# ayankele/dune-transformercvn

Hardware: AMD Instinct MI355X
Metric: events/sec (fwd+bwd) at batch=32, 8 prongs/event; fraction of MFMA roofline (higher is better)
Workload: dtype bf16; 1 GPU; TransformerCVN DenseNet [3,6,12,6,3] g32, fwd+loss+bwd, batch 32/GPU, 8 prongs/event, 3x400x280 maps, 6-layer encoder, dropout 0.1; global_batch=32, parallelism=dp1, precision=bf16

## Files before the change

### dune-transformercvn_amd/csrc/densenet.hip

```cpp
#include <string>
#include <vector>
#include <cstring>

#include "tcvn_rows.h"
#include <cstdlib>
#include "densenet_plan.h"

using namespace tcvn;

namespace {
constexpr float kEps = 1e-5f, kMom = 0.1f;
}

int DenseNetPlan::add_slot(const std::string& name, long numel, int kind) {
    slots.push_back({name, numel, kind});
    return (int)slots.size() - 1;
}
BnSlots DenseNetPlan::add_bn(const std::string& p, int c) {
    BnSlots s;
    s.w = add_slot(p + ".weight", c, TCVN_SLOT_PARAM);
    s.b = add_slot(p + ".bias", c, TCVN_SLOT_PARAM);
    s.rm = add_slot(p + ".running_mean", c, TCVN_SLOT_BUFFER);
    s.rv = add_slot(p + ".running_var", c, TCVN_SLOT_BUFFER);
    s.nbt = add_slot(p + ".num_batches_tracked", 1, TCVN_SLOT_COUNTER);
// ... 23 lines not shown
            const std::string p = f + ".dense" + std::to_string(b + 1) + ".layers." + std::to_string(l);
            ls.n1 = add_bn(p + ".bottleneck_block.norm1", cin);
            ls.a1 = add_slot(p + ".bottleneck_block.relu1.weight", cin, TCVN_SLOT_PARAM);
            ls.w1 = add_slot(p + ".bottleneck_block.conv1.weight", (long)mid * cin, TCVN_SLOT_PARAM);
            ls.b1 = add_slot(p + ".bottleneck_block.conv1.bias", mid, TCVN_SLOT_PARAM);
            ls.n2 = add_bn(p + ".output_block.norm2", mid);
            ls.a2 = add_slot(p + ".output_block.relu2.weight", mid, TCVN_SLOT_PARAM);
            ls.w2 = add_slot(p + ".output_block.conv2.weight", (long)g * mid * 9, TCVN_SLOT_PARAM);
            ls.b2 = add_slot(p + ".output_block.conv2.bias", g, TCVN_SLOT_PARAM);
            ls.cin = cin;
            bg.layers.push_back(ls);
        }
        ch = bg.Ctot;
        if (b != cfg.n_blocks - 1) {
            const std::string p = f + ".transition" + std::to_string(b + 1);
            bg.has_trans = true;
            bg.tn = add_bn(p + ".norm", ch);
            bg.ta = add_slot(p + ".relu.weight", ch, TCVN_SLOT_PARAM);
            bg.tw = add_slot(p + ".conv.weight", (long)(ch / 2) * ch, TCVN_SLOT_PARAM);
            bg.tb = add_slot(p + ".conv.bias", ch / 2, TCVN_SLOT_PARAM);
            ch = ch / 2; h = h / 2; w = w / 2;
        }
        blocks.push_back(bg);
    }
    Cf = ch;
    nf = add_bn(f + ".final_norm", ch);
    s_af = add_slot(f + ".final_relu.weight", ch, TCVN_SLOT_PARAM);
    s_wl = add_slot("output_block.linear.weight", (long)cfg.out_dim * ch, TCVN_SLOT_PARAM);
    nl = add_bn("output_block.norm", cfg.out_dim);
    s_al = add_slot("output_block.relu.weight", cfg.out_dim, TCVN_SLOT_PARAM);
    data.assign(slots.size(), nullptr);
    grad.assign(slots.size(), nullptr);
    for (const auto& bg : blocks) path.emplace_back(bg.L);
}

DenseNetPlan::~DenseNetPlan() {
    if (d_desc) (void)hipFree(d_desc);
    if (d_undesc) (void)hipFree(d_undesc);
    if (side_st) {
        (void)hipStreamSynchronize(side_st);
        (void)hipStreamDestroy(side_st);
        (void)hipEventDestroy(ev_fork_a); (void)hipEventDestroy(ev_fork_b); (void)hipEventDestroy(ev_done[0]);
        (void)hipEventDestroy(ev_done[1]); (void)hipEventDestroy(ev_drain);
    }
}
int DenseNetPlan::ensure_side() {
    if (side_st) return 0;
    TCVN_CHECK(hipStreamCreateWithFlags(&side_st, hipStreamNonBlocking));
    hipEvent_t* evs[5] = {&ev_fork_a, &ev_fork_b, &ev_done[0], &ev_done[1], &ev_drain};
    for (hipEvent_t* e : evs) TCVN_CHECK(hipEventCreateWithFlags(e, hipEventDisableTiming));
    return 0;
}

namespace {
struct Bump {
    long off = 0;
    long take(long bytes) { long o = off; off += round_up(bytes, 256); return o; }
};
}

void DenseNetPlan::layout(int n, bool bwd, Layout& L) const {
    Bump b;
    const int mid = cfg.bn_size * cfg.growth;
    L.img = b.take((long)n * cfg.H * cfg.W * cfg.in_ch * esz);
    L.c0 = b.take((long)n * Hc * Wc * cfg.init_ch * esz);
    L.D.clear(); L.Y.clear(); L.bstatD.clear(); L.bstatY.clear(); L.YA.clear(); L.XA.clear(); L.XP.clear(); L.KM.clear();
// ... 446 lines not shown
        if (!p.fuse_ya) {
            ActArgs act{Y, mid, M, mid, a.sc, a.sh, a.sl, s.ws + L.YA[bi][l], mid};
            if ((rc = act_bf16(act, s.st))) return rc;
        }
        a.Aact = s.ws + L.YA[bi][l];
    }
    a.part = s.train ? s.part : nullptr;
    a.drop_p = s.train ? cfg.dropout : 0.f; a.seed = s.seed; a.stream_id = (uint32_t)(bi * 64 + l + 1);
    a.nblk = conv_fwd_nblk(a);
    if (p.lf2) {
        if (!a.act_fused) { fprintf(stderr, "tcvn: link-free norm2 without the in-LDS activation\n"); return -17; }
        a.lf = lf_link(s, ls.n2, isumY, 2L * mid, 0, mid, bstatY, M);
    }
    if (p.out_isum) { a.isum_out = isumD + 2 * ls.cin; a.isum_stride = 2L * bg.ld; }
    if (s.train && !L.KM[bi].empty()) a.keep_out = reinterpret_cast<uint32_t*>(s.ws + L.KM[bi][l]);
    if ((rc = conv_fwd(a, s.st))) return rc;
    fr = FreshStats{ls.cin, g, a.nblk, g, p.out_isum};
    return 0;
}

int DenseNetPlan::fwd_transition(const Step& s, int bi, FreshStats& fr) {
    const Layout& L = s.L;
    const BlockGeom& bg = blocks[bi];
    char* D = s.ws + L.D[bi];
    int rc;
    if ((rc = link_fresh(s, bg.has_trans ? bg.tn : nf, bi, fr))) return rc;
    if (!bg.has_trans) {
        const Tab t = tab(s.ws, L, nf);
        HeadPoolArgs a{cfg.mode, D, bg.ld, s.n, bg.H * bg.W, Cf, t.sc, t.sh, data[s_af], reinterpret_cast<float*>(s.ws + L.F)};
        return head_pool_fwd(a, s.st);
    }
    const BlockGeom& nb = blocks[bi + 1];
    fr = FreshStats{0, nb.C0, 0, bg.Ctot / 2, false};
    if (L.XP[bi] >= 0) {
        const Tab t = tab(s.ws, L, bg.tn);
        ActPoolArgs ap{D, bg.ld, s.n, bg.H, bg.W, bg.Ctot, t.sc, t.sh, data[bg.ta], s.ws + L.XP[bi], bg.ldp};
        if ((rc = cfg.mode == MODE_BF16 ? act_pool_bf16(ap, s.st) : act_pool_f32(ap, s.st))) return rc;
    }
    if (L.XP[bi] >= 0 && cfg.mode == MODE_BF16) {
        const WkEntry& ef = wk_find(bg.tw, 0, 1);
        GemmNtArgs ga{};
        ga.epi = EPI_FWD; ga.A = s.ws + L.XP[bi]; ga.lda = bg.ldp; ga.K = bg.ldp; ga.M = (long)s.n * nb.H * nb.W; ga.N = bg.Ctot / 2;
        ga.Wfrag = s.ws + L.wk + ef.off; ga.Kp = ef.Kp; ga.zeros = s.ws + L.zeros; ga.bias = data[bg.tb];
        ga.Out = s.ws + L.D[bi + 1]; ga.ldo = nb.ld; ga.n_off = 0; ga.part = s.train ? s.part : nullptr; ga.nblk = gemm_nt_nblk(ga);
        if ((rc = gemm_nt_bf16(ga, "k_gemm_nt_bf16<fwdtrans>", s.st))) return rc;
        fr.nblk = ga.nblk;
        return 0;
    }
    ConvFwdArgs a = trans_args(s, bi);
    a.part = s.train ? s.part : nullptr; a.nblk = conv_fwd_nblk(a);
    if ((rc = conv_fwd(a, s.st))) return rc;
    fr.nblk = a.nblk;
    return 0;
}

int DenseNetPlan::fwd_output(const Step& s, float* out, long out_ld) const {
    float* F = reinterpret_cast<float*>(s.ws + s.L.F);
    float* Z = reinterpret_cast<float*>(s.ws + s.L.Z);
    int rc;
    if ((rc = linear_fwd(F, Cf, data[s_wl], nullptr, Z, cfg.out_dim, s.n, cfg.out_dim, Cf, s.st))) return rc;
    float* hs = reinterpret_cast<float*>(s.ws + s.L.head_stat);
    RowsBnArgs r{};
    r.X = Z; r.ldx = cfg.out_dim; r.R = s.n; r.C = cfg.out_dim; r.gamma = data[nl.w]; r.beta = data[nl.b]; r.slope = data[s_al];
    r.running_mean = data[nl.rm]; r.running_var = data[nl.rv]; r.Y = out; r.ldy = out_ld;
    r.save_mean = hs; r.save_rstd = hs + cfg.out_dim; r.train = s.train; r.eps = kEps; r.momentum = kMom;
    r.drop_p = s.train ? cfg.dropout : 0.f; r.seed = s.seed; r.stream_id = 0x4000u;
// ... 2 lines not shown

int DenseNetPlan::tap(int n, const char* name, long* off, int* tn, int* th, int* tw, int* tc, int* tld, int* tes) const {
    Layout L;
    layout(n, false, L);
    std::string s(name);
    *tn = n; *tes = esz;
    if ((s == "img" || s == "conv0") && stem_path.sparse && n == last_n) return -1;
    if (s == "img") { *off = L.img; *th = cfg.H; *tw = cfg.W; *tc = cfg.in_ch; *tld = cfg.in_ch; return 0; }
    if (s == "conv0") { *off = L.c0; *th = Hc; *tw = Wc; *tc = cfg.init_ch; *tld = cfg.init_ch; return 0; }
    if (s == "condense") { *off = L.F; *th = 1; *tw = 1; *tc = Cf; *tld = Cf; *tes = 4; return 0; }
    if (s == "raw:wk") { *tn = *th = *tw = 1; *off = L.wk; *tc = *tld = (int)(wk_bytes() / esz); return 0; }
    if (s == "raw:tabs") { *tn = *th = *tw = 1; *off = L.tabs; *tc = *tld = (int)tab_floats(); *tes = 4; return 0; }
    if (s.rfind("raw:ystat", 0) == 0) {
        int b = 0, l = 0;
        if (sscanf(s.c_str(), "raw:ystat%d.%d", &b, &l) != 2) return -1;
        b -= 1;
        if (b < 0 || b >= (int)blocks.size() || l < 0 || l >= blocks[b].L) return -1;
        *tn = *th = *tw = 1; *off = L.bstatY[b][l]; *tc = *tld = 2 * cfg.bn_size * cfg.growth; *tes = 8; return 0;
    }
    if (s.rfind("raw:isumy", 0) == 0) {
        int b = 0, l = 0;
        if (sscanf(s.c_str(), "raw:isumy%d.%d", &b, &l) != 2) return -1;
        b -= 1;
        if (b < 0 || b >= (int)blocks.size() || l < 0 || l >= blocks[b].L || L.isumY.empty() || n != last_n || !path[b][l].lf2) return -1;
        *tn = *th = *tw = 1; *off = L.isumY[b][l]; *tc = *tld = LF_REP * 2 * cfg.bn_size * cfg.growth; *tes = 8; return 0;
    }
    if (s.rfind("raw:bstat", 0) == 0) {
        const int b = atoi(s.c_str() + 9) - 1;
        if (s == "raw:bstat0") { *tn = *th = *tw = 1; *off = L.bstat0; *tc = *tld = cfg.init_ch * 2; *tes = 8; return 0; }
        if (b < 0 || b >= (int)blocks.size()) return -1;
        *tn = *th = *tw = 1; *off = L.bstatD[b]; *tc = *tld = blocks[b].ld * 2; *tes = 8; return 0;
    }
    if (s == "output_linear") { *off = L.Z; *th = 1; *tw = 1; *tc = *tld = cfg.out_dim; *tes = 4; return 0; }
    if (s == "raw:grad1") {
        Layout Lb;
        layout(n, true, Lb);
        *off = Lb.G[0]; *th = blocks[0].H; *tw = blocks[0].W; *tc = blocks[0].Ctot; *tld = blocks[0].ld; return 0;
    }
    if (s == "raw:head_stat") { *tn = *th = *tw = 1; *off = L.head_stat; *tc = *tld = 2 * cfg.out_dim; *tes = 4; return 0; }
    if (s.rfind("dense", 0) == 0) {
        const int b = atoi(s.c_str() + 5) - 1;
        if (b < 0 || b >= (int)blocks.size()) return -1;
        *off = L.D[b]; *th = blocks[b].H; *tw = blocks[b].W; *tc = blocks[b].Ctot; *tld = blocks[b].ld;
        return 0;
    }
    if (s.rfind("bottleneck", 0) == 0) {
        int b = 0, l = 0;
        if (sscanf(s.c_str(), "bottleneck%d.%d", &b, &l) != 2) return -1;
        b -= 1;
        if (b < 0 || b >= (int)blocks.size() || l < 0 || l >= blocks[b].L) return -1;
        for (const auto& pb : path)
            for (const LayerPath& p : pb) if (n == last_n && p.fuse_ya) return -1;
        *off = L.Y[b][l]; *th = blocks[b].H; *tw = blocks[b].W; *tc = cfg.bn_size * cfg.growth; *tld = *tc;
        return 0;
    }
    if (s.rfind("xa", 0) == 0 || s.rfind("ya", 0) == 0) {
        int b = 0, l = 0;
        if (sscanf(s.c_str() + 2, "%d.%d", &b, &l) != 2) return -1;
        b -= 1;
        if (b < 0 || b >= (int)blocks.size() || l < 0 || l >= blocks[b].L) return -1;
        const bool xa = s[0] == 'x';
        if ((xa && (L.XA[b].empty() || L.XA[b][l] < 0)) || (!xa && L.YA[b].empty())) return -1;
        if (n == last_n && (xa ? path[b][l].raw1x1 : path[b][l].act_fused)) return -1;
        *off = xa ? L.XA[b][l] : L.YA[b][l]; *th = blocks[b].H; *tw = blocks[b].W;
        *tc = xa ? blocks[b].layers[l].cin : cfg.bn_size * cfg.growth; *tld = xa ? (int)round_up(*tc, 8) : *tc;
        return 0;
    }
    return -1;
}

// ... 55 lines not shown
```

### dune-transformercvn_amd/csrc/densenet_bwd.hip

```cpp
#include <cstring>
#include <vector>

#include <cstdlib>
#include "densenet_plan.h"
#include "tcvn_rows.h"

using namespace tcvn;

static int g_backward_overlap = 0;
bool tcvn::backward_overlap_enabled() { return g_backward_overlap != 0; }
void tcvn::set_backward_overlap(int on) { g_backward_overlap = on; }

#ifdef TCVN_DEBUG_KNOBS
static struct { int block, layer; float* dst; } g_pq_tap = {0, 0, nullptr};
extern "C" void tcvn_debug_pq_tap(int block, int layer, float* dst) { g_pq_tap = {block, layer, dst}; }
#endif

namespace {
constexpr float kEps = 1e-5f;
constexpr long kSlabBytes = 48L << 20;
constexpr long kSlab1GemmBytes = 64L << 20;
constexpr long kSlab1Bytes = 68L << 20;
constexpr long kSlabGemmBytes = 44L << 20;
struct Bump {
    long off;
    long take(long bytes) { long o = off; off += round_up(bytes, 256); return o; }
};
}

void DenseNetPlan::layout_bwd(int n, long start, long maxY, Layout& L) const {
    Bump b{start};
    const int mid = cfg.bn_size * cfg.growth;
    L.G.clear(); L.pqD.clear();
    long bpart = (long)std::max(pool0_bwd_grid(n, Hc, Wc), pool0_bwd_vec_grid(n, Hc, Wc)) * cfg.init_ch * 24;
    bpart = std::max(bpart, 1024L * cfg.init_ch * 24);
    bpart = std::max(bpart, (long)head_pool_bwd_grid(n) * Cf * 24);
    for (const auto& bg : blocks) {
        const long M = (long)n * bg.H * bg.W;
        L.G.push_back(b.take(M * bg.ld * esz));
        bpart = std::max(bpart, 512L * std::max(mid, bg.Ctot) * 24);
    }
    for (const auto& bg : blocks) L.pqD.push_back(b.take((long)bg.ld * 8));
    long gw = 0;
    for (const auto& e : wk_list())
        if (!e.transpose && !e.frag) gw += round_up((long)e.N * e.Kp * 4, 256);
    L.gwk = b.take(gw);
    L.zero_end = b.off;
    L.du = b.take(maxY * esz);
// ... 6 lines not shown
    L.pq0 = b.take((long)cfg.init_ch * 8);
    L.bpart = b.take(bpart);
    L.dF = b.take((long)n * Cf * 4);
    L.dZ = b.take((long)n * cfg.out_dim * 4);
    L.EY3.clear();
    for (const auto& bg : blocks) {
        std::vector<long> eys;
        if (cfg.mode == MODE_BF16 && cfg.growth == 32)
            for (int l = 0; l < bg.L; ++l) eys.push_back(b.take((long)n * bg.H * bg.W * 32 * esz));
        L.EY3.push_back(eys);
    }
    L.total = b.off;
}

bool DenseNetPlan::bwd1x1_fill(int bi, int l, long M, char* ws, const Layout& L, Bwd1x1Args& fa) const {
    static const bool no_fuse1 = TCVN_KNOB_SET("TCVN_NO_BWD1_FUSE");
    const BlockGeom& bg = blocks[bi];
    const LayerSlots& ls = bg.layers[l];
    const int mid = cfg.bn_size * cfg.growth;
    if (no_fuse1 || L.XA[bi][l] < 0 || mid != 128 || L.slab1 < 0 || cfg.mode != MODE_BF16) return false;
    const Tab t1 = tab(ws, L, ls.n1);
    const WkEntry& etf = wk_find(ls.w1, 1, 1);
    fa = Bwd1x1Args{};
    fa.DU = ws + L.du; fa.Y = ws + L.Y[bi][l]; fa.PY = reinterpret_cast<float*>(ws + L.pqY); fa.QY = fa.PY + mid; fa.M = M;
    fa.Xin = ws + L.D[bi]; fa.ldx = bg.ld; fa.cin = ls.cin;
    fa.sc = t1.sc; fa.sh = t1.sh; fa.sl = data[ls.a1]; fa.Gout = ws + L.G[bi]; fa.ldg = bg.ld;
    fa.Wfrag = ws + L.wk + etf.off; fa.Kp = etf.Kp; fa.zeros = ws + L.zeros; fa.part = reinterpret_cast<double*>(ws + L.bpart);
    fa.slab = reinterpret_cast<float*>(ws + L.slab1); fa.slab_bytes = kSlab1GemmBytes; fa.ldc = wk_find(ls.w1, 0).Kp;
    fa.tail = reinterpret_cast<float*>(ws + L.slab1 + kSlab1GemmBytes);
    fa.nblk = bwd1x1_fused_nblk(fa);
    return bwd1x1_fused_ok(fa);
}

float* DenseNetPlan::gw_of(const Step& s, int slot) const {
    long o = 0;
    for (const WkEntry& e : wk_cache) {
        if (e.transpose || e.frag) continue;
        if (e.slot == slot) return reinterpret_cast<float*>(s.ws + s.L.gwk + o);
        o += round_up((long)e.N * e.Kp * 4, 256);
    }
    return nullptr;
}

int DenseNetPlan::bwd_link(const Step& s, const BnSlots& bn, int nblk, const double* bstat, long count, float* P, float* Q, int acc, int a_slot) const {
    BnBwdLinkArgs a{s.part, nblk, bn.C, bstat, count, kEps, data[bn.w], grad[bn.w], grad[bn.b], grad[a_slot], P, Q, acc};
    return bn_bwd_link(a, s.st);
}

int DenseNetPlan::drain(Step& s) const {
    if (s.side_on && s.side_busy) {
        TCVN_CHECK(hipEventRecord(ev_drain, side_st));
        TCVN_CHECK(hipStreamWaitEvent(s.st, ev_drain, 0));
        s.side_busy = false;
    }
    s.seq = 0;
    return 0;
}

int DenseNetPlan::backward(int n, const float* d_out, long d_out_ld, char* ws, long ws_bytes, hipStream_t st, int bi_hi, int bi_lo) {
    if (!bound) return -11;
    if (bi_hi < 0) bi_hi = (int)blocks.size() - 1;
    if (bi_lo < 0 || bi_lo > bi_hi || bi_hi >= (int)blocks.size()) return -1;
    const bool first_part = bi_hi == (int)blocks.size() - 1, last_part = bi_lo == 0;
    if (n <= 0) return 0;
    if (n != last_n) { fprintf(stderr, "tcvn: densenet backward without matching forward\n"); return -13; }
    for (size_t i = 0; i < slots.size(); ++i)
// ... 72 lines not shown
    const BlockGeom& bg = blocks[bi];
    const int mode = cfg.mode;
    const long M = (long)s.n * bg.H * bg.W;
    char* D = s.ws + L.D[bi];
    char* G = s.ws + L.G[bi];
    float* P = reinterpret_cast<float*>(s.ws + L.pqD[bi]);
    float* Q = P + bg.ld;
    const double* bstatD = reinterpret_cast<const double*>(s.ws + L.bstatD[bi]);
    int rc;
    if (!bg.has_trans) {
        const Tab t = tab(s.ws, L, nf);
        HeadPoolBwdArgs a{mode, D, bg.ld, s.n, bg.H * bg.W, Cf, t.sc, t.sh, data[s_af], reinterpret_cast<float*>(s.ws + L.dF), G, bg.ld, s.part,
                          head_pool_bwd_grid(s.n)};
        if ((rc = head_pool_bwd(a, s.st))) return rc;
        return bwd_link(s, nf, a.nblk, bstatD, M, P, Q, 1, s_af);
    }
    const BlockGeom& nb = blocks[bi + 1];
    const long Mn = (long)s.n * nb.H * nb.W;
    const int Nt = bg.Ctot / 2;
    float* Pn = reinterpret_cast<float*>(s.ws + L.pqD[bi + 1]);
    float* Qn = Pn + nb.ld;
    const EffSrc e{s.ws + L.G[bi + 1], nb.ld, s.ws + L.D[bi + 1], nb.ld, 0, Nt, Pn, Qn, 0.f, 0, 0};
    const Tab t = tab(s.ws, L, bg.tn);
    const WkEntry& ef = wk_find(bg.tw, 0);
    if ((rc = drain(s))) return rc;
    if (L.XP[bi] >= 0 && mode == MODE_BF16) {
        const int Nt8 = (int)round_up(Nt, 8);
        SlabJob bias_job{};
        EffMatArgs em{e, Mn, s.ws + L.ey, Nt8, grad[bg.tb], reinterpret_cast<float*>(s.ws + L.slab + kSlabGemmBytes), &bias_job};
        if ((rc = eff_materialize_bf16(em, s.st))) return rc;
        GemmTnArgs gt{s.ws + L.ey, Nt8, Nt8, s.ws + L.XP[bi], bg.ldp, bg.ldp, Mn, gw_of(s, bg.tw), ef.Kp, s.ws + L.zeros,
                      reinterpret_cast<float*>(s.ws + L.slab), kSlabGemmBytes, Nt, bias_job};
        if ((rc = gemm_tn_bf16(gt, "k_gemm_tn_bf16<transition>", s.st))) return rc;
        const WkEntry& etf = wk_find(bg.tw, 1, 1);
        GemmNtArgs ga{};
        ga.epi = EPI_DGRAD_POOL; ga.A = s.ws + L.ey; ga.lda = Nt8; ga.K = Nt8; ga.M = Mn; ga.N = bg.Ctot;
        ga.Wfrag = s.ws + L.wk + etf.off; ga.Kp = etf.Kp; ga.zeros = s.ws + L.zeros;
        ga.Xin = D; ga.ldxin = bg.ld; ga.sc = t.sc; ga.sh = t.sh; ga.sl = data[bg.ta];
        ga.Gout = G; ga.ldgo = bg.ld; ga.g_write = 1; ga.H = nb.H; ga.W = nb.W; ga.Hin = bg.H; ga.Win = bg.W;
        ga.part = s.part; ga.nblk = gemm_nt_nblk(ga);
        if ((rc = gemm_nt_bf16(ga, "k_gemm_nt_bf16<dgradtrans>", s.st))) return rc;
        return bwd_link(s, bg.tn, ga.nblk, bstatD, M, P, Q, 1, bg.ta);
    }
    ConvWgradArgs w{};
    w.mode = mode; w.e = e; w.dWk = gw_of(s, bg.tw); w.dbias = grad[bg.tb];
    w.fa = trans_args(s, bi);
    if (L.XP[bi] >= 0) { w.slab = reinterpret_cast<float*>(s.ws + L.slab); w.slab_bytes = kSlabBytes; }
    if ((rc = conv_wgrad(w, s.st))) return rc;
    const WkEntry& et = wk_find(bg.tw, 1);
    ConvDgradArgs d{};
    d.mode = mode; d.dmode = DG_1X1_POOL; d.e = e; d.M = (int)Mn; d.N = bg.Ctot; d.Kp = et.Kp;
    d.H = nb.H; d.W = nb.W; d.Hin = bg.H; d.Win = bg.W; d.Wt = s.ws + L.wk + et.off;
    d.Xin = D; d.ldxin = bg.ld; d.sc = t.sc; d.sh = t.sh; d.sl = data[bg.ta];
    d.Gout = G; d.ldgo = bg.ld; d.accumulate = 1; d.part = s.part; d.nblk = conv_dgrad_nblk(d);
    if ((rc = conv_dgrad(d, s.st))) return rc;
    return bwd_link(s, bg.tn, d.nblk, bstatD, M, P, Q, 1, bg.ta);
}

int DenseNetPlan::bwd_layer(Step& s, int bi, int l) const {
    const Layout& L = s.L;
    const BlockGeom& bg = blocks[bi];
    const LayerSlots& ls = bg.layers[l];
    const LayerPath& p = path[bi][l];
    const int mode = cfg.mode, g = cfg.growth, mid = cfg.bn_size * cfg.growth;
    const long M = (long)s.n * bg.H * bg.W;
    hipStream_t st = s.st;
    char* D = s.ws + L.D[bi];
    char* G = s.ws + L.G[bi];
    float* P = reinterpret_cast<float*>(s.ws + L.pqD[bi]);
    float* Q = P + bg.ld;
    const double* bstatD = reinterpret_cast<const double*>(s.ws + L.bstatD[bi]);
    char* Y = s.ws + L.Y[bi][l];
    char* DU = s.ws + L.du;
    float* PY = reinterpret_cast<float*>(s.ws + L.pqY);
// ... 150 lines not shown
```

### dune-transformercvn_amd/csrc/densenet_plan.h

```cpp
#pragma once
#include <string>
#include <vector>

#include "../../include/tcvn_hip.h"
#include "tcvn_ops.h"

namespace tcvn {

struct BnSlots { int w = -1, b = -1, rm = -1, rv = -1, nbt = -1, C = 0, id = -1; };
struct LayerSlots { BnSlots n1, n2; int a1, w1, b1, a2, w2, b2, cin; };
struct BlockGeom {
    int H, W, C0, L, Ctot, ld;
    int ldp;
    std::vector<LayerSlots> layers;
    bool has_trans = false;
    BnSlots tn; int ta = -1, tw = -1, tb = -1;
};
struct WkEntry { int slot, N, Cin, taps, transpose, rows, Kp, frag; long off; };

struct Layout {
    long img, c0, bstat0, part, tabs, F, Z, head_stat, wk, fwd_end, total;
    std::vector<long> D, bstatD;
    std::vector<std::vector<long>> Y, bstatY, YA;
    std::vector<std::vector<long>> EY3;
    std::vector<std::vector<long>> KM;
    long zeros, ey, ey2, slab;
    long isum_bytes = 0;
    std::vector<long> isumD;
    std::vector<std::vector<long>> isumY;
    long slab1;
    long sact;
    long sidx;
    std::vector<std::vector<long>> XA;
    std::vector<long> XP;
    long du, du0, pq0, pqY, gwk, bpart, dF, dZ, zero_end;
    std::vector<long> G, pqD;
};

struct LayerPath {
    bool fuse_ya = false;
    bool raw1x1 = false;
    bool act_fused = false;
    bool lf2 = false;
    bool out_isum = false;
    bool keep_stored = false;
};
struct StemPath {
    bool sparse = false;
    bool act_skip = false;
};
struct Tab { float* sc; float* sh; };
struct FreshStats { int c0, n, nblk, ld; bool isum; };
struct Step {
    char* ws; const Layout& L; hipStream_t st; int n; bool train; uint64_t seed;
    double* part; bool lf_on;
    bool side_on; int seq; bool side_busy;
};

bool backward_overlap_enabled();
void set_backward_overlap(int on);

struct DenseNetPlan {
    tcvn_densenet_cfg cfg;
    int esz, Hc, Wc, Cf, n_bn = 0;
    std::vector<Slot> slots;
    std::vector<float*> data, grad;
    std::vector<BlockGeom> blocks;
    int s_w0, s_b0, s_a0, s_af, s_wl, s_al;
    BnSlots n0, nf, nl;
    std::vector<WkEntry> wk_cache;
    bool bound = false;
    bool fast1_ok(int cin) const;
    bool fastt_ok(int Ctot) const;
    bool fast3x3 = false;
    char* d_desc = nullptr; size_t desc_cap = 0; std::vector<char> h_desc;
    char* desc_ws = nullptr; long desc_total = 0; int n_pack = 0, n_bneval = 0;
    uint64_t last_seed = 0; int last_n = 0;
    const int32_t* last_coords = nullptr; long last_nnz = 0;
    const float* last_values = nullptr; int last_value_mode = 0; float last_noise = 0.f;
    std::vector<std::vector<LayerPath>> path;
    StemPath stem_path;
    bool sparse_stem_possible() const;
    hipStream_t side_st = nullptr; hipEvent_t ev_fork_a = nullptr, ev_fork_b = nullptr, ev_done[2] = {nullptr, nullptr}, ev_drain = nullptr;
    int ensure_side();
    char* d_undesc = nullptr; std::vector<char> h_undesc; char* undesc_ws = nullptr; long undesc_total = 0; int n_unpack = 0;

    explicit DenseNetPlan(const tcvn_densenet_cfg& c);
    ~DenseNetPlan();
    int add_slot(const std::string& name, long numel, int kind);
    BnSlots add_bn(const std::string& p, int c);
    void layout(int n, bool bwd, Layout& L) const;
    void layout_bwd(int n, long start, long maxY, Layout& L) const;
    long tab_floats() const;
    long tab_off(const BnSlots& s) const;
    long wk_bytes() const;
    std::vector<WkEntry> wk_list() const;
    const WkEntry& wk_find(int slot, int transpose, int frag = 0) const;
    const void* wk_frag(const char* ws, const Layout& L, int slot, int transpose) const;
    int bind(void* const* d, void* const* g);
    int upload_descs(char* ws, const Layout& L, hipStream_t st);
    int forward(int n, const int32_t* coords, const float* values, long nnz, int log_pixels, float noise_std, float* out,
                long out_ld, char* ws, long ws_bytes, int train, uint64_t seed, hipStream_t st);
    int backward(int n, const float* d_out, long d_out_ld, char* ws, long ws_bytes, hipStream_t st, int bi_hi = -1, int bi_lo = 0);
    int fwd_stem(const Step& s, const int32_t* coords, const float* values, long nnz, int log_pixels, float noise_std, FreshStats& fr);
    int fwd_layer(const Step& s, int bi, int l, FreshStats& fr);
    int fwd_transition(const Step& s, int bi, FreshStats& fr);
    int fwd_output(const Step& s, float* out, long out_ld) const;
    LayerPath layer_path(const Step& s, int bi, int l, const ConvFwdArgs& c3, Fwd1x1Args& f1) const;
    int link(const Step& s, const BnSlots& bn, int nblk, int part_ld, int c_new0, int n_new, double* bstat, long count,
             const long long* isum = nullptr, long isum_stride = 0) const;
    int link_fresh(const Step& s, const BnSlots& bn, int bi, const FreshStats& fr) const;
    LfLink lf_link(const Step& s, const BnSlots& bn, const long long* isum, long rep_stride, int c_new0, int n_new, double* bstat, long count) const;
    int bwd_output(const Step& s, const float* d_out, long d_out_ld) const;
    int bwd_transition(Step& s, int bi) const;
    int bwd_layer(Step& s, int bi, int l) const;
    int bwd_stem(const Step& s) const;
    int bwd_link(const Step& s, const BnSlots& bn, int nblk, const double* bstat, long count, float* P, float* Q, int acc, int a_slot) const;
    int drain(Step& s) const;
    float* gw_of(const Step& s, int slot) const;
    Tab tab(char* ws, const Layout& L, const BnSlots& bn) const;
    ConvFwdArgs conv0_args(const Step& s) const, trans_args(const Step& s, int bi) const;
    ConvFwdArgs conv1_args(const Step& s, int bi, int l) const, conv3_args(const Step& s, int bi, int l) const;
    StemSparseArgs stem_sparse_args(const Step& s, const int32_t* coords, const float* values, long nnz, int value_mode, float noise_std) const;
    bool bwd1x1_fill(int bi, int l, long M, char* ws, const Layout& L, Bwd1x1Args& fa) const;
    std::vector<int> unpack_first;
    int tap(int n, const char* name, long* off, int* tn, int* th, int* tw, int* tc, int* tld, int* tes) const;
};

}
```

### dune-transformercvn_amd/csrc/tcvn_ops.h

```cpp
#pragma once
#include "tcvn_common.h"
#include "bn_lf.h"

namespace tcvn {

enum AMode { A_1X1 = 0, A_1X1_POOL = 1, A_3X3 = 2, A_STEM = 3 };

struct ConvFwdArgs {
    int mode, amode;
    const void* A; long lda;
    int M, N, K, Kp;
    int C, H, W, Hin, Win;
    const float *sc, *sh, *sl;
    const void* Wk; const float* bias;
    void* Out; long ldo; int n_off;
    const void* Wfrag;
    const void* Aact;
    const void* zeros;
    double* part; int nblk;
    float drop_p; uint64_t seed; uint32_t stream_id;
    uint32_t* keep_out;
    int act_fused;
    LfLink lf;
    long long* isum_out; long isum_stride;
// ... 159 lines not shown
    const void* Wfrag; int Kp;
    const void* zeros;
    const float* bias; void* Out; long ldo; int n_off;
    const float *osc, *osh, *osl;
    const void* Xin; long ldxin; const float *sc, *sh, *sl;
    void* Gout; long ldgo;
    int g_write;
    int H, W, Hin, Win;
    double* part; int nblk;
};
int zero_pool_remainder(void* G, long ld, int n_img, int Hin, int Win, int Ho, int Wo, hipStream_t st);
bool gemm_nt_ok(const GemmNtArgs& a);
int gemm_nt_nblk(const GemmNtArgs& a);
int gemm_nt_bf16(const GemmNtArgs& a, const char* label, hipStream_t st);

struct Bwd1x1Args {
    const void* DU; const void* Y;
    const float *PY, *QY;
    long M;
    const void* Xin; long ldx; int cin;
    const float *sc, *sh, *sl;
    void* Gout; long ldg;
    const void* Wfrag; int Kp;
    const void* zeros;
    double* part; int nblk;
    float* slab; long slab_bytes; long ldc;
    float* tail;
};
bool bwd1x1_fused_ok(const Bwd1x1Args& a);
int bwd1x1_fused_nblk(const Bwd1x1Args& a);
int bwd1x1_fused_launch(const Bwd1x1Args& a, hipStream_t st);
int bwd1x1_fused_reduce(const Bwd1x1Args& a, float* dWk, float* dbias, const SlabJob* extra, hipStream_t st, const BnBwdLinkArgs* link = nullptr);

struct Fwd1x1Args {
    const void* Xin; long ldx; int cin;
    const float *sc, *sh, *sl;
    long M;
    const void* Wfrag; int Kp;
    const float* bias; void* Out;
    const float *osc, *osh, *osl;
    const void* zeros;
    double* part; int nblk;
    LfLink lf;
    long long* isum_out; long isum_stride;
};
bool fwd1x1_fused_ok(const Fwd1x1Args& a);
int fwd1x1_fused_nblk(const Fwd1x1Args& a);
int fwd1x1_fused(const Fwd1x1Args& a, hipStream_t st);

struct EffMatArgs { EffSrc e; long M; void* Out; long ldo; float* colsum; float* slab;
                    SlabJob* deferred; };
int eff_materialize_bf16(const EffMatArgs& a, hipStream_t st);

struct ActPoolArgs { const void* X; long ldx; int n_img, Hin, Win, C; const float *sc, *sh, *sl; void* Out; long ldo; };
int act_pool_bf16(const ActPoolArgs& a, hipStream_t st);
int act_pool_f32(const ActPoolArgs& a, hipStream_t st);

inline int stem_act_words(int Wc) { return (Wc + 31) >> 5; }
int stem_mark(const int* coords, long nnz, int n_img, int H, int W, int Hc, int Wc, uint32_t* act, const float* bias, void* cline, hipStream_t st);
int pool0_bwd_vec_grid(int n_img, int Hin, int Win);
bool pool0_bwd_vec_ok(const Pool0BwdArgs& a);
int pool0_bwd_vec(const Pool0BwdArgs& a, hipStream_t st);
struct StemWgradArgs {
    const int* coords; long nnz; const void* img; int n_img, H, W, Cpix;
    EffSrc e;
    int Hc, Wc, Kp; float* slab; long slab_bytes;
// ... 37 lines not shown
```

Before: 1797 events/s.

## Add dedicated fused transition data-gradient kernel with register-resident weights

Adds a specialized kernel for the transition-layer backward data gradient. It keeps the 1x1 conv weight fragments in registers, double-buffers ET and X tiles through shared memory, and fuses the avg-pool scatter, PReLU/BN backward and the per-block stat partials. The forward pass records whether this path is eligible, and the backward pass uses it in place of the generic gemm_nt dgrad-pool epilogue. The intent is to cut the generic GEMM's overhead and memory traffic for these skinny-K GEMMs. The cost is extra code, a fixed grid cap and a changed partial-sum layout handed to bwd_link.

```diff
diff --git a/dune-transformercvn_amd/csrc/densenet.hip b/dune-transformercvn_amd/csrc/densenet.hip
--- a/dune-transformercvn_amd/csrc/densenet.hip
+++ b/dune-transformercvn_amd/csrc/densenet.hip
@@ -79,6 +79,7 @@
     data.assign(slots.size(), nullptr);
     grad.assign(slots.size(), nullptr);
     for (const auto& bg : blocks) path.emplace_back(bg.L);
+    tpath.assign(blocks.size(), TransPath{});
 }
 
 DenseNetPlan::~DenseNetPlan() {
@@ -591,6 +592,8 @@
     }
     const BlockGeom& nb = blocks[bi + 1];
     fr = FreshStats{0, nb.C0, 0, bg.Ctot / 2, false};
+    TransBwdArgs tb{};
+    tpath[bi].dgrad_tile = s.train && trans_bwd_fill(bi, s.n, s.ws, L, tb);
     if (L.XP[bi] >= 0) {
         const Tab t = tab(s.ws, L, bg.tn);
         ActPoolArgs ap{D, bg.ld, s.n, bg.H, bg.W, bg.Ctot, t.sc, t.sh, data[bg.ta], s.ws + L.XP[bi], bg.ldp};
@@ -659,10 +662,12 @@
         *tn = *th = *tw = 1; *off = L.bstatD[b]; *tc = *tld = blocks[b].ld * 2; *tes = 8; return 0;
     }
     if (s == "output_linear") { *off = L.Z; *th = 1; *tw = 1; *tc = *tld = cfg.out_dim; *tes = 4; return 0; }
-    if (s == "raw:grad1") {
+    if (s.rfind("raw:grad", 0) == 0) {
+        const int b = atoi(s.c_str() + 8) - 1;
+        if (b < 0 || b >= (int)blocks.size()) return -1;
         Layout Lb;
         layout(n, true, Lb);
-        *off = Lb.G[0]; *th = blocks[0].H; *tw = blocks[0].W; *tc = blocks[0].Ctot; *tld = blocks[0].ld; return 0;
+        *off = Lb.G[b]; *th = blocks[b].H; *tw = blocks[b].W; *tc = blocks[b].Ctot; *tld = blocks[b].ld; return 0;
     }
     if (s == "raw:head_stat") { *tn = *th = *tw = 1; *off = L.head_stat; *tc = *tld = 2 * cfg.out_dim; *tes = 4; return 0; }
     if (s.rfind("dense", 0) == 0) {
diff --git a/dune-transformercvn_amd/csrc/densenet_bwd.hip b/dune-transformercvn_amd/csrc/densenet_bwd.hip
--- a/dune-transformercvn_amd/csrc/densenet_bwd.hip
+++ b/dune-transformercvn_amd/csrc/densenet_bwd.hip
@@ -14,6 +14,10 @@
 #ifdef TCVN_DEBUG_KNOBS
 static struct { int block, layer; float* dst; } g_pq_tap = {0, 0, nullptr};
 extern "C" void tcvn_debug_pq_tap(int block, int layer, float* dst) { g_pq_tap = {block, layer, dst}; }
+static int g_trans_grid_cap = 0;
+extern "C" void tcvn_debug_trans_grid_cap(int cap) { g_trans_grid_cap = cap > 0 ? cap : 0; }
+static struct { int block; void* g; void* et; float* tab; double* part; int* nblk; } g_trans_tap = {-1, nullptr, nullptr, nullptr, nullptr, nullptr};
+extern "C" void tcvn_debug_trans_tap(int block, void* g, void* et, float* tab, double* part, int* nblk_out) { g_trans_tap = {block, g, et, tab, part, nblk_out}; }
 #endif
 
 namespace {
@@ -86,6 +90,27 @@
     return bwd1x1_fused_ok(fa);
 }
 
+bool DenseNetPlan::trans_bwd_fill(int bi, int n, char* ws, const Layout& L, TransBwdArgs& ta) const {
+    static const bool no_fuse = TCVN_KNOB_SET("TCVN_NO_TRANS_FUSE");
+    const BlockGeom& bg = blocks[bi];
+    if (no_fuse || !bg.has_trans || cfg.mode != MODE_BF16 || L.XP[bi] < 0 || L.G.empty()) return false;
+    const BlockGeom& nb = blocks[bi + 1];
+    const int Nt8 = (int)round_up(bg.Ctot / 2, 8);
+    const Tab t = tab(ws, L, bg.tn);
+    const WkEntry& etf = wk_find(bg.tw, 1, 1);
+    ta = TransBwdArgs{};
+    ta.ET = ws + L.ey; ta.lde = Nt8; ta.K = Nt8; ta.M = (long)n * nb.H * nb.W; ta.N = bg.Ctot;
+    ta.Wfrag = ws + L.wk + etf.off; ta.Kp = etf.Kp;
+    ta.Xin = ws + L.D[bi]; ta.ldx = bg.ld; ta.sc = t.sc; ta.sh = t.sh; ta.sl = data[bg.ta];
+    ta.Gout = ws + L.G[bi]; ta.ldg = bg.ld; ta.H = nb.H; ta.W = nb.W; ta.Hin = bg.H; ta.Win = bg.W;
+    ta.part = reinterpret_cast<double*>(ws + L.bpart);
+#ifdef TCVN_DEBUG_KNOBS
+    ta.grid_cap = g_trans_grid_cap;
+#endif
+    ta.nblk = trans_dgrad_nblk(ta);
+    return trans_dgrad_ok(ta);
+}
+
 float* DenseNetPlan::gw_of(const Step& s, int slot) const {
     long o = 0;
     for (const WkEntry& e : wk_cache) {
@@ -224,6 +249,28 @@
         GemmTnArgs gt{s.ws + L.ey, Nt8, Nt8, s.ws + L.XP[bi], bg.ldp, bg.ldp, Mn, gw_of(s, bg.tw), ef.Kp, s.ws + L.zeros,
                       reinterpret_cast<float*>(s.ws + L.slab), kSlabGemmBytes, Nt, bias_job};
         if ((rc = gemm_tn_bf16(gt, "k_gemm_tn_bf16<transition>", s.st))) return rc;
+#ifdef TCVN_DEBUG_KNOBS
+        auto tap_out = [&](int nblk) -> int {
+            if (g_trans_tap.block != bi) return 0;
+            if (g_trans_tap.g) TCVN_CHECK(hipMemcpyAsync(g_trans_tap.g, G, (size_t)(M * bg.ld * esz), hipMemcpyDeviceToDevice, s.st));
+            if (g_trans_tap.et) TCVN_CHECK(hipMemcpyAsync(g_trans_tap.et, s.ws + L.ey, (size_t)(Mn * Nt8 * esz), hipMemcpyDeviceToDevice, s.st));
+            if (g_trans_tap.tab) {
+                TCVN_CHECK(hipMemcpyAsync(g_trans_tap.tab, t.sc, (size_t)bg.Ctot * 4, hipMemcpyDeviceToDevice, s.st));
+                TCVN_CHECK(hipMemcpyAsync(g_trans_tap.tab + bg.Ctot, t.sh, (size_t)bg.Ctot * 4, hipMemcpyDeviceToDevice, s.st));
+            }
+            if (g_trans_tap.part) TCVN_CHECK(hipMemcpyAsync(g_trans_tap.part, s.part, (size_t)nblk * bg.Ctot * 24, hipMemcpyDeviceToDevice, s.st));
+            if (g_trans_tap.nblk) *g_trans_tap.nblk = nblk;
+            return 0;
+        };
+#else
+        auto tap_out = [](int) { return 0; };
+#endif
+        if (tpath[bi].dgrad_tile) {
+            TransBwdArgs ta{};
+            if (!trans_bwd_fill(bi, s.n, s.ws, L, ta)) { fprintf(stderr, "tcvn: transition %d: the recorded data-gradient path cannot run\n", bi); return -15; }
+            if ((rc = trans_dgrad_launch(ta, s.st)) || (rc = tap_out(ta.nblk))) return rc;
+            return bwd_link(s, bg.tn, ta.nblk, bstatD, M, P, Q, 1, bg.ta);
+        }
         const WkEntry& etf = wk_find(bg.tw, 1, 1);
         GemmNtArgs ga{};
         ga.epi = EPI_DGRAD_POOL; ga.A = s.ws + L.ey; ga.lda = Nt8; ga.K = Nt8; ga.M = Mn; ga.N = bg.Ctot;
@@ -231,7 +278,7 @@
         ga.Xin = D; ga.ldxin = bg.ld; ga.sc = t.sc; ga.sh = t.sh; ga.sl = data[bg.ta];
         ga.Gout = G; ga.ldgo = bg.ld; ga.g_write = 1; ga.H = nb.H; ga.W = nb.W; ga.Hin = bg.H; ga.Win = bg.W;
         ga.part = s.part; ga.nblk = gemm_nt_nblk(ga);
-        if ((rc = gemm_nt_bf16(ga, "k_gemm_nt_bf16<dgradtrans>", s.st))) return rc;
+        if ((rc = gemm_nt_bf16(ga, "k_gemm_nt_bf16<dgradtrans>", s.st)) || (rc = tap_out(ga.nblk))) return rc;
         return bwd_link(s, bg.tn, ga.nblk, bstatD, M, P, Q, 1, bg.ta);
     }
     ConvWgradArgs w{};
diff --git a/dune-transformercvn_amd/csrc/densenet_plan.h b/dune-transformercvn_amd/csrc/densenet_plan.h
--- a/dune-transformercvn_amd/csrc/densenet_plan.h
+++ b/dune-transformercvn_amd/csrc/densenet_plan.h
@@ -49,6 +49,9 @@
     bool sparse = false;
     bool act_skip = false;
 };
+struct TransPath {
+    bool dgrad_tile = false;
+};
 struct Tab { float* sc; float* sh; };
 struct FreshStats { int c0, n, nblk, ld; bool isum; };
 struct Step {
@@ -80,6 +83,7 @@
     const float* last_values = nullptr; int last_value_mode = 0; float last_noise = 0.f;
     std::vector<std::vector<LayerPath>> path;
     StemPath stem_path;
+    std::vector<TransPath> tpath;
     bool sparse_stem_possible() const;
     hipStream_t side_st = nullptr; hipEvent_t ev_fork_a = nullptr, ev_fork_b = nullptr, ev_done[2] = {nullptr, nullptr}, ev_drain = nullptr;
     int ensure_side();
@@ -123,6 +127,7 @@
     ConvFwdArgs conv1_args(const Step& s, int bi, int l) const, conv3_args(const Step& s, int bi, int l) const;
     StemSparseArgs stem_sparse_args(const Step& s, const int32_t* coords, const float* values, long nnz, int value_mode, float noise_std) const;
     bool bwd1x1_fill(int bi, int l, long M, char* ws, const Layout& L, Bwd1x1Args& fa) const;
+    bool trans_bwd_fill(int bi, int n, char* ws, const Layout& L, TransBwdArgs& ta) const;
     std::vector<int> unpack_first;
     int tap(int n, const char* name, long* off, int* tn, int* th, int* tw, int* tc, int* tld, int* tes) const;
 };
diff --git a/dune-transformercvn_amd/csrc/tcvn_ops.h b/dune-transformercvn_amd/csrc/tcvn_ops.h
--- a/dune-transformercvn_amd/csrc/tcvn_ops.h
+++ b/dune-transformercvn_amd/csrc/tcvn_ops.h
@@ -215,6 +215,21 @@
 int bwd1x1_fused_launch(const Bwd1x1Args& a, hipStream_t st);
 int bwd1x1_fused_reduce(const Bwd1x1Args& a, float* dWk, float* dbias, const SlabJob* extra, hipStream_t st, const BnBwdLinkArgs* link = nullptr);
 
+struct TransBwdArgs {
+    const void* ET; long lde; int K;
+    long M; int N;
+    const void* Wfrag; int Kp;
+    const void* Xin; long ldx;
+    const float *sc, *sh, *sl;
+    void* Gout; long ldg;
+    int H, W, Hin, Win;
+    double* part; int nblk;
+    int grid_cap;
+};
+bool trans_dgrad_ok(const TransBwdArgs& a);
+int trans_dgrad_nblk(const TransBwdArgs& a);
+int trans_dgrad_launch(const TransBwdArgs& a, hipStream_t st);
+
 struct Fwd1x1Args {
     const void* Xin; long ldx; int cin;
     const float *sc, *sh, *sl;
diff --git a/dune-transformercvn_amd/csrc/trans_bwd_fused.hip b/dune-transformercvn_amd/csrc/trans_bwd_fused.hip
--- /dev/null
+++ b/dune-transformercvn_amd/csrc/trans_bwd_fused.hip
@@ -0,0 +1,277 @@
+#include <type_traits>
+#include "tcvn_ops.h"
+#include "prof.h"
+
+namespace tcvn {
+
+namespace {
+
+typedef __attribute__((ext_vector_type(4))) unsigned u32x4;
+constexpr int ROWS = 32;
+constexpr int CLD = 132;
+constexpr int KCH = ROWS * 256;
+constexpr int KS_SMALL = 10, NKC_SMALL = 2;
+constexpr int KS_WIDE = 18, NKC_WIDE = 3;
+
+constexpr int OFF_X = 0;
+constexpr int OFF_A = OFF_X + 8 * 256 * 16;
+template <int NKC> constexpr int smem_bytes() { return OFF_A + NKC * KCH + ROWS * CLD * 4 + 3 * 128 * 4; }
+
+template <int NKC>
+__device__ __forceinline__ void load_a(u32x4 (&av)[NKC][ROWS / 16], const bf16* __restrict__ A, long lda, int K, int nkc, long m0, long M, int wave, int lane) {
+    const int rsub = lane >> 4, slot = lane & 15;
+#pragma unroll
+    for (int kc = 0; kc < NKC; ++kc)
+#pragma unroll
+        for (int i = 0; i < ROWS / 16; ++i) {
+            const int r = (wave + 4 * i) * 4 + rsub;
+            const int col = kc * 128 + ((slot ^ (r & 15)) << 3);
+            const long m = m0 + r;
+            av[kc][i] = u32x4{0u, 0u, 0u, 0u};
+            if (kc < nkc && m < M && col < K) av[kc][i] = *reinterpret_cast<const u32x4*>(A + m * lda + col);
+        }
+}
+template <int NKC>
+__device__ __forceinline__ void store_a(char* abuf, const u32x4 (&av)[NKC][ROWS / 16], int nkc, int wave, int lane) {
+#pragma unroll
+    for (int kc = 0; kc < NKC; ++kc)
+        if (kc < nkc)
+#pragma unroll
+            for (int i = 0; i < ROWS / 16; ++i) *reinterpret_cast<u32x4*>(abuf + kc * KCH + (wave + 4 * i) * 1024 + lane * 16) = av[kc][i];
+}
+
+template <int MAXKS, int NKC>
+__global__ __launch_bounds__(256, 2) void k_trans_dgrad_bf16(const TransBwdArgs g) {
+    extern __shared__ __attribute__((aligned(16))) char smem[];
+    constexpr int OFF_C = OFF_A + NKC * KCH;
+    float* Cs = reinterpret_cast<float*>(smem + OFF_C);
+    double* red = reinterpret_cast<double*>(smem + OFF_C);
+    float* tab = reinterpret_cast<float*>(smem + OFF_C + ROWS * CLD * 4);
+
+    const int tid = threadIdx.x;
+    const int n0 = blockIdx.y * 128;
+    const bf16* __restrict__ A = reinterpret_cast<const bf16*>(g.ET);
+    const bf16* __restrict__ Xp = reinterpret_cast<const bf16*>(g.Xin);
+    bf16* __restrict__ Gp = reinterpret_cast<bf16*>(g.Gout);
+    const int ksteps = g.Kp >> 4, nkc = (g.K + 127) >> 7;
+    const long mtiles = (g.M + ROWS - 1) / ROWS;
+    const u16x8 z8 = {0, 0, 0, 0, 0, 0, 0, 0};
+
+    const bool wave_live = n0 + (tid >> 6) * 32 < g.N;
+    bf16x8_t bw[MAXKS];
+    {
+        const bf16* __restrict__ Wf = reinterpret_cast<const bf16*>(g.Wfrag) + (((long)(blockIdx.y * 4 + (tid >> 6)) * ksteps) * 64 + (tid & 63)) * 8;
+#pragma unroll
+        for (int i = 0; i < MAXKS; ++i)
+            if (i < ksteps && wave_live) bw[i] = *reinterpret_cast<const bf16x8_t*>(Wf + (long)i * 512);
+            else
+#pragma unroll
+                for (int j = 0; j < 8; ++j) bw[i][j] = (__bf16)0.f;
+    }
+    if (tid < 128) {
+        const bool ok = n0 + tid < g.N;
+        tab[tid] = ok ? g.sc[n0 + tid] : 0.f; tab[128 + tid] = ok ? g.sh[n0 + tid] : 0.f; tab[256 + tid] = ok ? g.sl[n0 + tid] : 0.f;
+    }
+    const int hw = g.H * g.W;
+    constexpr bool DIRECT = MAXKS > KS_SMALL;
+    typedef typename std::conditional<DIRECT, float, double>::type stat_t;
+    stat_t st1[8], st2[8], st3[8];
+#pragma unroll
+    for (int j = 0; j < 8; ++j) { st1[j] = 0; st2[j] = 0; st3[j] = 0; }
+
+    auto request_x = [&](long t, int c_r0, int ncol, u16x8 (&xv)[ROWS / 16][4], int (&px)[ROWS / 16]) {
+#pragma unroll
+        for (int i = 0; i < ROWS / 16; ++i) {
+            const unsigned m = (unsigned)t * ROWS + c_r0 + 16 * i;
+            const unsigned mm = m < (unsigned)g.M ? m : (unsigned)g.M - 1;
+            const unsigned img = mm / (unsigned)hw;
+            const unsigned rem = mm - img * hw;
+            const unsigned ho = rem / (unsigned)g.W, wo = rem - ho * g.W;
+            px[i] = (int)((img * g.Hin + 2 * ho) * g.Win + 2 * wo);
+            if (ncol < g.N) {
+#pragma unroll
+                for (int q = 0; q < 4; ++q)
+                    xv[i][q] = *reinterpret_cast<const u16x8*>(Xp + (long)(px[i] + (q >> 1) * g.Win + (q & 1)) * g.ldx + ncol);
+            }
+        }
+    };
+    u16x8 xn[ROWS / 16][4];
+    int pn[ROWS / 16], pc[ROWS / 16];
+#pragma unroll
+    for (int i = 0; i < ROWS / 16; ++i) {
+        pn[i] = 0; pc[i] = 0;
+#pragma unroll
+        for (int q = 0; q < 4; ++q) xn[i][q] = z8;
+    }
+
+    long mt = blockIdx.x;
+    u32x4 an[NKC][ROWS / 16];
+    if (mt < mtiles) {
+        load_a<NKC>(an, A, g.lde, g.K, nkc, mt * ROWS, g.M, tid >> 6, tid & 63);
+        request_x(mt, tid >> 4, n0 + (tid & 15) * 8, xn, pn);
+    }
+    for (; mt < mtiles; mt += gridDim.x) {
+        int t_o = tid;
+        asm volatile("" : "+v"(t_o));
+        const int lane = t_o & 63, wave = t_o >> 6;
+        const int r = lane & 31, h = lane >> 5;
+        const int c8 = t_o & 15, c_r0 = t_o >> 4;
+        const int ncol = n0 + c8 * 8;
+        const bool col_ok = ncol < g.N;
+        const int col_rem = g.N - ncol;
+        u16x8* xs = reinterpret_cast<u16x8*>(smem + OFF_X) + t_o;
+        asm volatile("s_waitcnt vmcnt(0)" ::: "memory");
+        store_a<NKC>(smem + OFF_A, an, nkc, wave, lane);
+#pragma unroll
+        for (int i = 0; i < ROWS / 16; ++i) {
+            pc[i] = pn[i];
+#pragma unroll
+            for (int q = 0; q < 4; ++q) xs[(4 * i + q) * 256] = xn[i][q];
+        }
+        __syncthreads();
+        const long nt = mt + gridDim.x;
+        if (nt < mtiles) {
+            request_x(nt, c_r0, ncol, xn, pn);
+            load_a<NKC>(an, A, g.lde, g.K, nkc, nt * ROWS, g.M, wave, lane);
+        }
+        __builtin_amdgcn_sched_barrier(0);
+        f32x16 acc;
+#pragma unroll
+        for (int e = 0; e < 16; ++e) acc[e] = 0.f;
+        {
+            const char* ab = smem + OFF_A + r * 256;
+#pragma unroll
+            for (int kc = 0; kc < NKC; ++kc) {
+                if (kc < nkc) {
+#pragma unroll
+                    for (int ks = 0; ks < 8; ++ks) {
+                        if (kc * 8 + ks < MAXKS && kc * 8 + ks < ksteps) {
+                            const bf16x8_t a = *reinterpret_cast<const bf16x8_t*>(ab + kc * KCH + (((2 * ks + h) ^ (r & 15)) << 4));
+                            acc = __builtin_amdgcn_mfma_f32_32x32x16_bf16(a, bw[kc * 8 + ks < MAXKS ? kc * 8 + ks : 0], acc, 0, 0, 0);
+                        }
+                    }
+                }
+            }
+        }
+#pragma unroll
+        for (int e = 0; e < 16; ++e) Cs[((e & 3) + 8 * (e >> 2) + 4 * h) * CLD + wave * 32 + r] = acc[e];
+        __syncthreads();
+        if (col_ok) {
+            float csc[8], csh[8], csl[8];
+            {
+                const float4 a0 = *reinterpret_cast<const float4*>(tab + c8 * 8), a1 = *reinterpret_cast<const float4*>(tab + c8 * 8 + 4);
+                const float4 b0 = *reinterpret_cast<const float4*>(tab + 128 + c8 * 8), b1 = *reinterpret_cast<const float4*>(tab + 128 + c8 * 8 + 4);
+                const float4 d0 = *reinterpret_cast<const float4*>(tab + 256 + c8 * 8), d1 = *reinterpret_cast<const float4*>(tab + 256 + c8 * 8 + 4);
+                csc[0] = a0.x; csc[1] = a0.y; csc[2] = a0.z; csc[3] = a0.w; csc[4] = a1.x; csc[5] = a1.y; csc[6] = a1.z; csc[7] = a1.w;
+                csh[0] = b0.x; csh[1] = b0.y; csh[2] = b0.z; csh[3] = b0.w; csh[4] = b1.x; csh[5] = b1.y; csh[6] = b1.z; csh[7] = b1.w;
+                csl[0] = d0.x; csl[1] = d0.y; csl[2] = d0.z; csl[3] = d0.w; csl[4] = d1.x; csl[5] = d1.y; csl[6] = d1.z; csl[7] = d1.w;
+            }
+            float t1[DIRECT ? 1 : 8], t2[DIRECT ? 1 : 8], t3[DIRECT ? 1 : 8];
+            float* const f1 = DIRECT ? reinterpret_cast<float*>(st1) : t1;
+            float* const f2 = DIRECT ? reinterpret_cast<float*>(st2) : t2;
+            float* const f3 = DIRECT ? reinterpret_cast<float*>(st3) : t3;
+            if (!DIRECT)
+#pragma unroll
+                for (int j = 0; j < 8; ++j) { f1[j] = 0.f; f2[j] = 0.f; f3[j] = 0.f; }
+#pragma unroll 1
+            for (int p = 0; p < 4 * (ROWS / 16); ++p) {
+                const int rr = c_r0 + 16 * (p >> 2), q = p & 3;
+                if (mt * ROWS + rr >= g.M) break;
+                const float4 ca = *reinterpret_cast<const float4*>(Cs + rr * CLD + c8 * 8);
+                const float4 cc = *reinterpret_cast<const float4*>(Cs + rr * CLD + c8 * 8 + 4);
+                const float cv[8] = {ca.x, ca.y, ca.z, ca.w, cc.x, cc.y, cc.z, cc.w};
+                bf16* gp = Gp + (long)((p >> 2 ? pc[1] : pc[0]) + (q >> 1) * g.Win + (q & 1)) * g.ldg + ncol;
+                u16x8 xv = xs[p * 256];
+                if (col_rem < 8) {
+#pragma unroll
+                    for (int j = 0; j < 8; ++j) xv[j] = j < col_rem ? xv[j] : (bf16)0;
+                }
+                u16x8 o;
+#pragma unroll
+                for (int j = 0; j < 8; ++j) {
+                    const float x = bf2f(xv[j]);
+                    const float u = fmaf(x, csc[j], csh[j]);
+                    const float dA = 0.25f * cv[j];
+                    const float du = u > 0.f ? dA : csl[j] * dA;
+                    f1[j] += du; f2[j] += du * x; f3[j] += u > 0.f ? 0.f : dA * u;
+                    o[j] = f2bf(csc[j] * du);
+                }
+                if (col_rem >= 8) *reinterpret_cast<u16x8*>(gp) = o;
+                else {
+#pragma unroll
+                    for (int j = 0; j < 8; ++j)
+                        if (j < col_rem) gp[j] = o[j];
+                }
+            }
+            if (!DIRECT)
+#pragma unroll
+                for (int j = 0; j < 8; ++j) { st1[j] += (stat_t)f1[j]; st2[j] += (stat_t)f2[j]; st3[j] += (stat_t)f3[j]; }
+        }
+    }
+    asm volatile("s_waitcnt vmcnt(0)" ::: "memory");
+    if (g.part == nullptr) return;
+    const int lane = tid & 63, wave = tid >> 6, c8 = tid & 15;
+    __syncthreads();
+#pragma unroll
+    for (int j = 0; j < 8; ++j) {
+        double d1 = (double)st1[j], d2 = (double)st2[j], d3 = (double)st3[j];
+        d1 += __shfl_xor(d1, 16); d1 += __shfl_xor(d1, 32);
+        d2 += __shfl_xor(d2, 16); d2 += __shfl_xor(d2, 32);
+        d3 += __shfl_xor(d3, 16); d3 += __shfl_xor(d3, 32);
+        if (lane < 16) {
+            double* p = red + ((wave * 128) + c8 * 8 + j) * 3;
+            p[0] = d1; p[1] = d2; p[2] = d3;
+        }
+    }
+    __syncthreads();
+    if (tid < 128 && n0 + tid < g.N) {
+        double a = 0, b = 0, c = 0;
+#pragma unroll
+        for (int w = 0; w < 4; ++w) { a += red[(w * 128 + tid) * 3]; b += red[(w * 128 + tid) * 3 + 1]; c += red[(w * 128 + tid) * 3 + 2]; }
+        double* p = g.part + ((long)blockIdx.x * g.N + n0 + tid) * 3;
+        p[0] = a; p[1] = b; p[2] = c;
+    }
+}
+
+bool wide(const TransBwdArgs& a) { return a.Kp > KS_SMALL * 16; }
+
+}
+
+bool trans_dgrad_ok(const TransBwdArgs& a) {
+    if (!a.ET || !a.Wfrag || !a.Xin || !a.Gout || !a.sc || !a.sh || !a.sl || !a.part) return false;
+    if (a.M <= 0 || a.N <= 0 || a.K <= 0 || (a.lde & 7) || (a.K & 7) || a.K > a.lde || (a.Kp & 15) || a.Kp < a.K || a.Kp > KS_WIDE * 16) return false;
+    if ((a.ldx & 7) || (a.ldg & 7) || a.N > a.ldx || a.N > a.ldg) return false;
+    if (a.H <= 0 || a.W <= 0 || a.Hin < 2 * a.H || a.Win < 2 * a.W || a.M % ((long)a.H * a.W) != 0) return false;
+    if (a.M / ((long)a.H * a.W) * a.Hin * a.Win >= (1L << 31)) return false;
+    const uintptr_t al = reinterpret_cast<uintptr_t>(a.ET) | reinterpret_cast<uintptr_t>(a.Wfrag) | reinterpret_cast<uintptr_t>(a.Xin) |
+                         reinterpret_cast<uintptr_t>(a.Gout);
+    return (al & 15) == 0 && a.grid_cap >= 0;
+}
+
+int trans_dgrad_nblk(const TransBwdArgs& a) {
+    int cap = (int)(512L * 128 / a.N);
+    if (cap < 64) cap = 64;
+    if (cap > 512) cap = 512;
+    if (a.grid_cap > 0 && a.grid_cap < cap) cap = a.grid_cap;
+    const long mt = (a.M + ROWS - 1) / ROWS;
+    return (int)(mt < cap ? mt : cap);
+}
+
+int trans_dgrad_launch(const TransBwdArgs& a, hipStream_t st) {
+    if (!trans_dgrad_ok(a)) return -2;
+    if (a.nblk != trans_dgrad_nblk(a)) { fprintf(stderr, "tcvn: trans_dgrad nblk mismatch\n"); return -3; }
+    static bool attr = false;
+    if (!attr) {
+        TCVN_CHECK(hipFuncSetAttribute(reinterpret_cast<const void*>(k_trans_dgrad_bf16<KS_SMALL, NKC_SMALL>), hipFuncAttributeMaxDynamicSharedMemorySize, 80 * 1024));
+        TCVN_CHECK(hipFuncSetAttribute(reinterpret_cast<const void*>(k_trans_dgrad_bf16<KS_WIDE, NKC_WIDE>), hipFuncAttributeMaxDynamicSharedMemorySize, 80 * 1024));
+        attr = true;
+    }
+    ProfScope ps("k_trans_dgrad_bf16", 2.0 * a.M * (double)a.N * a.K, (double)a.M * 2.0 * (a.K + 8.0 * a.N), st);
+    const dim3 grid(a.nblk, cdiv(a.N, 128));
+    if (wide(a)) hipLaunchKernelGGL((k_trans_dgrad_bf16<KS_WIDE, NKC_WIDE>), grid, dim3(256), smem_bytes<NKC_WIDE>(), st, a);
+    else hipLaunchKernelGGL((k_trans_dgrad_bf16<KS_SMALL, NKC_SMALL>), grid, dim3(256), smem_bytes<NKC_SMALL>(), st, a);
+    TCVN_LAUNCH_CHECK();
+    return 0;
+}
+
+}
```

Measured after the change: 1804 events/s, median of 2. Within noise of the previous version (+0.4%).
